# floswald/SMM.jl

Measured on AMD Instinct MI355X. Metric: chain-evals/sec (whole node), serialNormal 2p/2m, 4096 chains x 200 iters, higher is better.
Workload: dtype f64

## Files before the change

### smm.jl_amd/csrc/smm_chain_persist.hpp

```cpp
#pragma once
constexpr int PR_K = 8;
constexpr int PR_ZR = 20;
constexpr int PR_MAX_ITERS = 4000;
constexpr int PR_GATHER_DELAY = 8;
constexpr int PR_STW = 12;
constexpr unsigned long long PERSIST_TMO_FIRST = 40000000ull;

__host__ __device__ inline int persist_line(int np) { return PR_STW + ((3 + 2 * np + 1) & ~1); }

struct PrWin { uint32_t ctl, arrive, fin, progress, slot, rec; size_t total; };
__host__ __device__ inline PrWin pr_win_layout(const int Ng, const int RW, const int G, const int tiles_rank) {
    PrWin L;
    size_t o = 0;
    L.ctl = (uint32_t)o; o += 128;
    L.arrive = (uint32_t)o; o += (size_t)128 * P2P_MAXG;
    L.fin = (uint32_t)o; o += (size_t)128 * P2P_MAXG;
    L.progress = (uint32_t)o; o += (((size_t)G * tiles_rank * 4) + 127) & ~(size_t)127;
    L.slot = (uint32_t)o; o += ((size_t)PR_K * ((size_t)Ng + 4) * 8 + 127) & ~(size_t)127;
    L.rec = (uint32_t)o; o += ((size_t)PR_K * (size_t)Ng * RW * 16 + 127) & ~(size_t)127;
    L.total = o;
    return L;
}

struct PersistArgs {
// ... 9 lines not shown
    int ring_k, slow_tile, slow_ticks, walk_first, unit_sh, scout_after, scout_gl;
    uint32_t epoch;
    double sigma_adjust_by, thr;
    uint64_t seed;
    unsigned long long tmo;
    const double* mi_g;
    int u_lanes, n_udata;
    unsigned char* win[P2P_MAXG];
    uint32_t o_arrive;
    int G, rank, offset;
    int slow_read;
    uint32_t o_slot;
    int tables_local;
    const double* chol_L;
    int chol_per_chain;
};

__device__ inline uint32_t pr_tag16(const uint32_t epoch, const int rel) { return 0x8000u | ((epoch & 0x7fu) << 8) | ((uint32_t)rel & 0xffu); }
__device__ inline uint32_t pr_tag32(const uint32_t epoch, const int rel) { return 0x80000000u | ((epoch & 0x7ffffu) << 12) | ((uint32_t)rel & 0xfffu); }
__device__ inline uint32_t pr_progress_word(const uint32_t epoch, const int rel) { return (epoch << 12) | (uint32_t)rel; }

#define PR_SC "sc0 sc1"
__device__ inline unsigned long long pr_load8_sys(const void* p) {
    unsigned long long v;
    asm volatile("global_load_dwordx2 %0, %1, off " PR_SC "\n\ts_waitcnt vmcnt(0)" : "=v"(v) : "v"(p) : "memory");
    return v;
}
__device__ inline uint32_t pr_load4_sys(const void* p) { return __hip_atomic_load((const uint32_t*)p, __ATOMIC_RELAXED, __HIP_MEMORY_SCOPE_SYSTEM); }
__device__ inline uint4 pr_load16_sys(const void* p) {
    p2p_u32x4 q;
// ... 238 lines not shown
```

### smm.jl_amd/csrc/smm_chain_persist_loc.hpp

```cpp
#pragma once
constexpr int PL_LOCN = NORM_CT + CONE_GCAP + 2;
constexpr uint32_t PL_PBASE = ((16u * PL_LOCN + 127u) & ~127u);
constexpr int PL_HASH = 1024;
constexpr size_t PL_TSW_BASE = (size_t)8 * 8192;
constexpr int PL_TSW_TILES = 2048, PL_TSW = 8;
constexpr size_t PL_LATE_BASE = PL_TSW_BASE + (size_t)PL_TSW_TILES * (NORM_WG / 64) * PL_TSW;
constexpr int PL_LATE_N = 16384;
static_assert(PL_LATE_BASE + PL_LATE_N <= (size_t)8 * 60000, "the stamp buffer: the exchange kernels' words start at 8 * 60000");

__host__ __device__ inline size_t persist_loc_smem_bytes(const int np) {
    const size_t hw = (size_t)((H_PARAMS + 2 * np + 1) & ~1);
    const size_t dbl = (size_t)NORM_CT * np + (size_t)np * 8 * NORM_CT + (size_t)NORM_CT * persist_line(np) + 2 * 64 * (size_t)(1 + 2 * np) +
                       2 * NORM_CT * hw + (size_t)PR_ZR * 64 + 16 + 16 + 2 * 64 * 2 + (size_t)PL_LOCN * np + (size_t)PL_LOCN +
                       (size_t)(NORM_WG / 64) * PL_TSW;
    return (size_t)PL_PBASE + 2 * (size_t)CONE_LEVELS * 64 * 4 + 2 * (size_t)CONE_GCAP * 2 + 4 * 16 * 4 + 2 * (size_t)PL_HASH * 4 + dbl * 8;
}

template <int NP>
struct PersistLocLds {
    using L = NormLayout<NP>;
    static constexpr int CT = NORM_CT, RW = L::RW, HW = L::HW, LW = PR_STW + RW, RNGW = 1 + 2 * NP;
    uint32_t pbase, gbase, hbase, tbase;
    uint32_t* s_hdr;
    double *s_theta, *s_part, *s_st, *s_rng, *s_hrow, *s_xrow, *s_z0, *s_const, *s_gth, *s_thr;
    uint4* s_donor;
    unsigned long long *s_ts, *s_wts;
    unsigned* s_arrived; int* s_minprog; unsigned* s_abort; unsigned* s_xmask; int* s_glready; int* s_pub; int* s_hready;
    __device__ inline PersistLocLds(unsigned char* lds) {
        pbase = PL_PBASE;
        gbase = pbase + 2u * CONE_LEVELS * 64 * 4;
        hbase = gbase + 2u * CONE_GCAP * 2;
        tbase = hbase + 4u * 16 * 4;
        s_hdr = (uint32_t*)(lds + hbase);
        s_theta = (double*)(lds + tbase + 2u * PL_HASH * 4);
        s_part = s_theta + CT * NP;
        s_st = s_part + NP * 8 * CT;
        s_rng = s_st + CT * LW;
        s_hrow = s_rng + 2 * 64 * RNGW;
        s_xrow = s_hrow + CT * HW;
        s_z0 = s_xrow + CT * HW;
        s_const = s_z0 + PR_ZR * 64;
        s_ts = (unsigned long long*)(s_const + 16);
        s_arrived = (unsigned*)(s_ts + 8);
        s_minprog = (int*)(s_arrived + 1);
        s_abort = s_arrived + 2;
        s_xmask = s_arrived + 3;
        s_glready = (int*)(s_arrived + 4);
        s_pub = (int*)(s_arrived + 5);
        s_hready = (int*)(s_arrived + 6);
        s_donor = (uint4*)(s_const + 16 + 16);
        s_gth = s_const + 16 + 16 + 2 * 64 * 2;
        s_thr = s_gth + PL_LOCN * NP;
        s_wts = (unsigned long long*)(s_thr + PL_LOCN);
    }
};

__device__ inline uint32_t pl_hslot(const uint32_t chain) { return (chain * 2654435761u) >> 22; }
static_assert(PL_HASH == 1024, "pl_hslot: 10 bits");
__device__ inline void pl_hash_put(uint32_t* tab, const uint32_t chain, const uint32_t local) {
    uint32_t h = pl_hslot(chain);
    while (atomicCAS(&tab[h], 0u, ((chain + 1u) << 16) | local) != 0u) h = (h + 1u) & (PL_HASH - 1);
}
__device__ inline uint32_t pl_hash_get(const uint32_t* tab, const uint32_t chain) {
    uint32_t h = pl_hslot(chain);
    for (int probe = 0; probe < PL_HASH; ++probe) {
        const uint32_t v = tab[h];
        if ((v >> 16) == chain + 1u) return v & 0xffffu;
        if (v == 0u) break;
// ... 86 lines not shown
                for (int k = 0; k < NP; ++k) Y.s_gth[cl * NP + k] = A.rec_in[(size_t)c * RW + 3 + k];
                if constexpr (PCT) Y.s_thr[cl] = A.mi_g[c0g + (uint32_t)cl];
            }
        }
#pragma unroll
        for (int u = 0; u < PR_ZR; ++u) Y.s_z0[u * 64 + lane] = (lane + u * WG < A.ns) ? A.Z[lane + (size_t)u * WG] : 0.0;
    }
    if (tid >= 64 && tid < 64 + NP) {
        const int k = tid - 64;
        Y.s_const[k] = A.lb[k]; Y.s_const[NP + k] = A.ub[k]; Y.s_const[2 * NP + k] = A.mom[k]; Y.s_const[3 * NP + k] = A.w[k];
    }
    if (tid == 128) {
        Y.s_const[4 * NP] = A.failbox ? A.objp[0] : 1.0; Y.s_const[4 * NP + 1] = A.failbox ? A.objp[1] : 0.0;
        Y.s_const[4 * NP + 2] = (double)A.ns;
        *Y.s_arrived = 0u; *Y.s_minprog = 0; *Y.s_abort = 0u; *Y.s_xmask = 0u; *Y.s_glready = t0 - 2; *Y.s_pub = t0 - 2; *Y.s_hready = t0 - 2;
    }
    if (tid >= 192 && tid < 200) Y.s_ts[tid - 192] = 0ull;
    if (A.ts && tid >= 256 && tid < 256 + (NORM_WG / 64) * PL_TSW) Y.s_wts[tid - 256] = 0ull;
    if (wave == 3 && lane < CONE_HDRW) {
        if (A.walk_first) Y.s_hdr[((t0 - 1) & 3) * 16 + lane] = A.cone_hdr[((size_t)(t0 - 1 - A.plan_t0) * tiles + tile) * CONE_HDRW + lane];
        if (t0 < t1 && exch_on(t0)) Y.s_hdr[(t0 & 3) * 16 + lane] = A.cone_hdr[((size_t)(t0 - A.plan_t0) * tiles + tile) * CONE_HDRW + lane];
    }
    if constexpr (SH) {
        if (tile == 0 && wave == 2 && lane < A.G) {
            unsigned char* w = nullptr;
#pragma unroll
            for (int p = 0; p < P2P_MAXG; ++p) w = lane == p ? A.win[p] : w;
            __hip_atomic_store((uint32_t*)(w + A.o_arrive + 128 * (size_t)A.rank), epoch, __ATOMIC_RELAXED, __HIP_MEMORY_SCOPE_SYSTEM);
        }
        if (wave == 2) {
// ... 222 lines not shown
        };
        if (wave == 1 || (wave == 2 && PR_AHEAD > 1)) make_rng(t0, wave - 1);
        for (int t = t0; t <= t1; ++t) {
            const int rel = t - t0 + 1;
            PR_BARRIER();
            uint32_t nhdr = 0u;
            const bool want_hdr = wave == 3 && lane < CONE_HDRW && t + 1 < t1 && exch_on(t + 1);
            if (wave == 3) {
                if (t > t0) {
                    store_rows(Y.s_hrow, t - 1, 0xffffu);
                    store_rows(Y.s_xrow, t - 2, *Y.s_xmask);
                }
                if (want_hdr) nhdr = A.cone_hdr[((size_t)(t + 1 - A.plan_t0) * tiles + tile) * CONE_HDRW + lane];
            }
            if (t < t1 && exch_on(t)) request_lists(t);
            PR_BARRIER();
            unsigned long long tw0 = 0, tw1 = 0, tw2 = 0;
            if (A.ts) tw0 = wall_clock64();
            if (simw) {
                __builtin_amdgcn_s_setprio(1);
                if (nfull == PR_ZR - 1) persist_simulate<NP, true>(z, nfull, extra, Y.s_theta, Y.s_part, h, wih, A.ts != nullptr, tw1);
                else persist_simulate<NP, false>(z, nfull, extra, Y.s_theta, Y.s_part, h, wih, A.ts != nullptr, tw1);
                if (A.ts) tw2 = wall_clock64();
                __builtin_amdgcn_fence(__ATOMIC_RELEASE, "workgroup");
                const int lane3 = (int)__builtin_amdgcn_mbcnt_hi(~0u, __builtin_amdgcn_mbcnt_lo(~0u, 0u));
                if (lane3 == 0) __hip_atomic_fetch_add(Y.s_arrived, 1u, __ATOMIC_RELAXED, __HIP_MEMORY_SCOPE_WORKGROUP);
                __builtin_amdgcn_s_setprio(0);
            }
            const int lane = (int)__builtin_amdgcn_mbcnt_hi(~0u, __builtin_amdgcn_mbcnt_lo(~0u, 0u));
            const bool lists = t < t1 && exch_on(t);
            if (wave == 3 || wave >= 8) {
                if (wave == 3 && want_hdr) Y.s_hdr[((t + 1) & 3) * 16 + lane] = nhdr;
                asm volatile("s_waitcnt vmcnt(0)" ::: "memory");
                if (wave == 3 && lane == 0) __hip_atomic_store(Y.s_glready, t, __ATOMIC_RELEASE, __HIP_MEMORY_SCOPE_WORKGROUP);
                if (wave == 3 && lists) {
                    build_table(t, lane);
                    if (lane == 0) __hip_atomic_store(Y.s_hready, t, __ATOMIC_RELEASE, __HIP_MEMORY_SCOPE_WORKGROUP);
                }
                if (wave >= 8 && lists) {
                    if (!A.tables_local) while (__hip_atomic_load(Y.s_hready, __ATOMIC_ACQUIRE, __HIP_MEMORY_SCOPE_WORKGROUP) != t) __builtin_amdgcn_s_sleep(1);
                    fix_lists(t, t + 1, lane);
                }
            }
            if (wave == 2) {
                const int m = pr_min_progress(pr_progress, epoch, tiles_all, lane);
                if (lane == 0) {
                    __hip_atomic_store(Y.s_minprog, m, __ATOMIC_RELAXED, __HIP_MEMORY_SCOPE_WORKGROUP);
                    if (pr_load4_sys(pr_ctl) == epoch) *Y.s_abort = 1u;
                    if (lists && A.cone_ok[t - A.plan_t0] == 0u) pr_report(A.err, 3, t + 1, (int)c0g);
                }
                if constexpr (SH) {
                    if (*Y.s_abort && lane < A.G) {
                        unsigned char* w = nullptr;
#pragma unroll
                        for (int p = 0; p < P2P_MAXG; ++p) w = lane == p ? A.win[p] : w;
                        __hip_atomic_store((uint32_t*)(w + A.o_ctl), epoch, __ATOMIC_RELAXED, __HIP_MEMORY_SCOPE_SYSTEM);
// ... 22 lines not shown
                const double2* st2 = (const double2*)(Y.s_st + cl * LW);
                double2* g_cs = (double2*)(A.cs + (size_t)c * CSW);
                for (int i = r; i < 6; i += 4) g_cs[i] = i == 2 ? make_double2(st2[2].x, 0.0) : st2[i];
                for (int i = r; i < NPC; i += 4) ((double2*)(A.rec_out + (size_t)c * RW))[i] = st2[PR_STW / 2 + i];
                if (r == 0) {
                    const double v = Y.s_st[cl * LW + PR_STW];
                    A.vals_out[c] = v;
                    if (A.slot8_out) { A.slot8_out[c] = make_uint2(order_key32(v), (uint32_t)c); if (v != v) atomicOr(A.walk_flags, 1u); }
                }
            }
        }
        return;
    }

    const int nfull0 = A.ns / WG;
    for (int t = t0; t <= t1; ++t) {
        const int rel = t - t0 + 1;
        const bool exch = t == t0 ? A.walk_first != 0 : exch_on(t - 1);
        double z0[PR_ZR];
        uint32_t wmeta;
        PR_BARRIER();
        {
            const int lane = (int)__builtin_amdgcn_mbcnt_hi(~0u, __builtin_amdgcn_mbcnt_lo(~0u, 0u));
            const int cl = lane >> 2, r = lane & 3;
            const int c = tile * CT + cl;
            const bool valid = c < N;
            double* st = Y.s_st + cl * LW;
            unsigned long long ts1 = 0;
            if (A.ts && lane == 0) { ts1 = wall_clock64(); if (t != t0) Y.s_ts[0] += ts1 - Y.s_ts[7]; }
            wmeta = (uint32_t)cl;
            if (exch) {
                const uint32_t lbase = Y.pbase + (uint32_t)((t - 1) & 1) * (CONE_LEVELS * 64 * 4);
                uint32_t hw, pw0;
                lean_sub64_head(Y.hbase + (uint32_t)((t - 1) & 3) * 64u, lbase, lane, hw, pw0);
                const int nsub = (int)((uint32_t)__builtin_amdgcn_readfirstlane((int)hw) & 0xffffu);
                if constexpr (WIDE) {
                    lean_walk_sub64<0, true, WalkNoGuard, PCT>(lbase, nsub, lane, pw0, A.thr, WalkNoGuard(), (uint32_t)((unsigned char*)Y.s_thr - lds));
                } else {
                    const PersistLocWalkValues values{W, mine, A.o_rec, rel, rmask, A.Ng, Y.gbase + (uint32_t)((t - 1) & 1) * (CONE_GCAP * 2), c0g, RW, NP, t};
                    lean_walk_sub64<0, false, PersistLocWalkValues>(lbase, nsub, lane, pw0, 0.0, values);
                }
                if (valid) wmeta = WIDE ? ((const uint4*)lds)[cl].z : ((const uint2*)lds)[cl].y;
            }
            const uint32_t src = wmeta & 0xffffu;
            const bool donor = valid && src != (uint32_t)cl;
            unsigned long long ts2 = 0;
            if (A.ts && lane == 0) ts2 = wall_clock64();
            double mu01[NP], th[NP], th_old[NP];
            const double sigma = st[CS_SIGMA];
            const double* o = Y.s_rng + ((t & 1) * 64 + lane) * RNGW;
            bool found = !valid;
            {
                double x[NP];
                bool ok = valid;
#pragma unroll
                for (int k = 0; k < NP; ++k) {
                    const double lbk = Y.s_const[k], ubk = Y.s_const[NP + k];
                    th_old[k] = donor ? Y.s_gth[src * NP + k] : st[PR_STW + 3 + k];
                    th[k] = valid ? th_old[k] : 0.0;
                    mu01[k] = (th_old[k] - lbk) / (ubk - lbk);
                    const double step = sigma * o[1 + k];
                    x[k] = mu01[k] + step;
                    if (!(x[k] >= 0.0 && x[k] <= 1.0)) ok = false;
                }
                if (r >= A.smpl_iters || (A.user_n && r >= A.rb_tries)) ok = false;
                const unsigned long long m = __ballot(ok);
                const unsigned quad = (unsigned)(m >> (lane & ~3)) & 0xfu;
                if (quad) {
                    const int rwin = __builtin_ctz(quad);
#pragma unroll
                    for (int k = 0; k < NP; ++k) {
                        const double lbk = Y.s_const[k];
                        const double sc = x[k] * (Y.s_const[NP + k] - lbk);
                        const double thk = sc + lbk;
                        th[k] = quad_bcast_dyn(thk, lane, rwin);
                    }
                    found = true;
                }
            }
            if (__builtin_expect(__any(!found), 0)) {
                if (A.ts && lane == 0) Y.s_wts[7] -= wall_clock64();
                int j_next = NORM_NR;
                if (PR_AHEAD > 1 && (A.rb == nullptr || A.rb_tries >= 2 * NORM_NR)) {
                    double x[NP];
                    bool ok = !found;
#pragma unroll
                    for (int k = 0; k < NP; ++k) {
                        const double step = sigma * o[1 + NP + k];
                        x[k] = mu01[k] + step;
                        if (!(x[k] >= 0.0 && x[k] <= 1.0)) ok = false;
                    }
                    if (NORM_NR + r >= A.smpl_iters || (A.user_n && NORM_NR + r >= A.rb_tries)) ok = false;
                    const unsigned long long m = __ballot(ok);
                    const unsigned quad = (unsigned)(m >> (lane & ~3)) & 0xfu;
                    if (!found && quad) {
                        const int rwin = __builtin_ctz(quad);
#pragma unroll
                        for (int k = 0; k < NP; ++k) {
                            const double lbk = Y.s_const[k];
                            const double sc = x[k] * (Y.s_const[NP + k] - lbk);
                            const double thk = sc + lbk;
                            th[k] = quad_bcast_dyn(thk, lane, rwin);
                        }
                        found = true;
                    }
                    j_next = 2 * NORM_NR;
                }
                if (__any(!found)) {
                    const PrTries TR{A.rb, A.seed, A.rb_t0, A.N, A.RBW, A.rb_tries, A.user_n, A.smpl_iters, A.offset};
                    const PrTh<NP> lt = persist_late_tries<NP>(TR, o, t, c, valid, lane, found, sigma, mu01[0], mu01[NP - 1], Y.s_const, th[0], th[NP - 1], j_next);
#pragma unroll
                    for (int k = 0; k < NP; ++k) th[k] = lt.th[k];
                    found = lt.found;
                    if (!found && r == 0) pr_report(A.err, ERRK_NO_DRAW, t, (int)c0g + cl);
                }
                if (A.ts && lane == 0) {
// ... 57 lines not shown
            __builtin_amdgcn_s_setprio(0);
        }
        {
            const unsigned want = (unsigned)(8 * NP) * (unsigned)rel;
            while (__hip_atomic_load(Y.s_arrived, __ATOMIC_RELAXED, __HIP_MEMORY_SCOPE_WORKGROUP) < want) __builtin_amdgcn_s_sleep(1);
            __builtin_amdgcn_fence(__ATOMIC_ACQUIRE, "workgroup");
        }
        if (A.ts) tw3 = wall_clock64();
        const int lane = (int)__builtin_amdgcn_mbcnt_hi(~0u, __builtin_amdgcn_mbcnt_lo(~0u, 0u));
        const int cl = lane >> 2, r = lane & 3;
        const int c = tile * CT + cl;
        const bool valid = c < N;
        double* st = Y.s_st + cl * LW;
        unsigned long long ts5 = 0;
        if (A.ts && lane == 0) ts5 = wall_clock64();
        if (valid) {
            const int src = (int)st[CS_WASX];
            const bool donor = src != cl;
            double rc2[RW];
#pragma unroll
            for (int f = 0; f < RW; ++f) rc2[f] = st[PR_STW + f];
            if (donor) {
                asm volatile("s_waitcnt vmcnt(0)" ::: "memory");
                const uint32_t tag = pr_tag32(epoch, rel - 1);
                double rr[8];
#pragma unroll
                for (int f = 0; f < 8; ++f) rr[f] = 0.0;
                bool ok = true;
#pragma unroll
                for (int f = 0; f < RW; ++f) {
// ... 63 lines not shown
                if (r == 0) {
                    double* hx = Y.s_xrow + cl * HW;
                    swapped_head(hx, rc2, partner, b);
#pragma unroll
                    for (int k = 0; k < 2 * NP; ++k) hx[H_PARAMS + k] = rc2[3 + k];
                    if (HW > H_PARAMS + 2 * NP) hx[HW - 1] = 0.0;
                }
            } else { nn += 1; na += (int)st[CS_LACC]; }
            double nsig = sig;
            const bool upd = (t % A.sigma_update_steps) == 0;
            if (upd || t == t1) {
                const double rate = accept_rate(na, nn, acc);
                if (upd) nsig = sigma_next(sig, rate, A.sigma_adjust_by);
                if (r == 0) st[CS_RATE] = rate;
            }
            const double currv = acc ? value : old;
            const Best b = best_of(value, t, bp, bpid);
            const double bestv = b.best, bestid = b.best_id;
            if (r == 0) {
                if constexpr (WIDE) ((uint4*)lds)[cl] = make_uint4((uint32_t)__double2loint(v), (uint32_t)__double2hiint(v), (uint32_t)cl, 0u);
                else ((uint2*)lds)[cl] = make_uint2(order_key32(v), (uint32_t)cl);
#pragma unroll
                for (int k = 0; k < NP; ++k) Y.s_gth[cl * NP + k] = nr[3 + k];
                st[CS_SIGMA] = nsig; st[CS_NNOEX] = (double)nn; st[CS_NACC] = (double)na; st[CS_LACC] = accd;
                st[CS_BEST] = bestv; st[CS_BESTID] = bestid; st[CS_BESTP] = bp; st[CS_BESTPID] = bpid;
#pragma unroll
                for (int f = 0; f < RW; ++f) st[PR_STW + f] = nr[f];
                double* hv = Y.s_hrow + cl * HW;
                history_head(hv, value, prob, currv, bestv, bestid, 0.0, accd, (double)status);
#pragma unroll
// ... 3 lines not shown
        }
        {
            const unsigned long long xm = __ballot(valid && r == 0 && (int)st[CS_PARTNER] != 0);
            if (lane == 0) {
                unsigned m = 0u;
#pragma unroll
                for (int q = 0; q < CT; ++q) m |= (unsigned)((xm >> (4 * q)) & 1ull) << q;
                *Y.s_xmask = m;
            }
        }
        if (A.ts && lane == 0) { const unsigned long long ts7 = wall_clock64(); Y.s_ts[2] += ts7 - Y.s_ts[6]; Y.s_ts[7] = ts7; pl_wts_add(Y.s_wts, tw0, tw1, tw2, tw3); }
    }
    PR_BARRIER();
    {
        const int lane = (int)__builtin_amdgcn_mbcnt_hi(~0u, __builtin_amdgcn_mbcnt_lo(~0u, 0u));
        if (A.ts && lane < 7) A.ts[(size_t)tile * 8 + lane] = lane < 6 ? Y.s_ts[lane] : (unsigned long long)(t1 - t0 + 1);
        if (A.ts && lane == 0) pl_wts_out(A.ts, Y.s_wts, tile, 0);
    }
}
```

### smm.jl_amd/csrc/smm_run_host.hpp

```cpp
#pragma once

namespace {

void persist_repair(Ctx* c, int n_replay = -1);
void p2p_enqueue(Ctx* c, int n_iters);
unsigned long long p2p_agree_error(Ctx* c, unsigned long long e_local) {
    const KParams& P = c->P;
    const int G = P.p2p_G;
    const PrWin WL = pr_win_layout(P.Ng, P.RW, G, persist_tiles_rank(c->F, c->P.N));
    const uint32_t seq = c->pr_epoch;
    for (int r = 0; r < G; ++r)
        HIPCHK(hipMemcpy(P.p2p_win[r] + c->prw_off + WL.fin + 128 * (size_t)P.p2p_rank, &e_local, 8, hipMemcpyHostToDevice));
    for (int r = 0; r < G; ++r)
        HIPCHK(hipMemcpy(P.p2p_win[r] + c->prw_off + WL.fin + 128 * (size_t)P.p2p_rank + 8, &seq, 4, hipMemcpyHostToDevice));
    std::vector<unsigned char> buf((size_t)128 * G);
    const auto t0 = std::chrono::steady_clock::now();
    unsigned long long e = e_local;
    for (;;) {
        HIPCHK(hipMemcpy(buf.data(), c->p2p_mine + c->prw_off + WL.fin, buf.size(), hipMemcpyDeviceToHost));
        bool all = true;
        e = e_local;
        for (int r = 0; r < G; ++r) {
            uint32_t s_r; unsigned long long e_r;
            memcpy(&e_r, buf.data() + 128 * (size_t)r, 8); memcpy(&s_r, buf.data() + 128 * (size_t)r + 8, 4);
// ... 187 lines not shown
        for (int r = 0; r < G; ++r) A.win[r] = P.p2p_win[r] + c->prw_off;
        A.self = c->p2p_mine + c->prw_off;
    } else { A.win[0] = c->prw; A.self = c->prw; }
    A.o_ctl = WL.ctl; A.o_arrive = WL.arrive; A.o_progress = WL.progress; A.o_slot = WL.slot; A.o_rec = WL.rec;
    A.cs = P.cs; A.rec_in = c->rec[c->run.cur]; A.rec_out = c->rec[c->run.cur ^ 1]; A.vals_out = P.vals_out; A.slot8_out = P.slot8_out; A.walk_flags = P.walk_flags;
    A.hrec = P.hrec; A.err = P.err; A.ts = P.ts;
    A.Z = P.Z; A.lb = P.lb; A.ub = P.ub; A.mom = P.mom; A.w = P.w; A.objp = P.objp; A.dense_Bf = P.dense_Bf; A.dense_Af = P.dense_Af; A.dense_A2f = P.dense_A2f;
    A.rb = pregen ? P.rb : nullptr;
    A.mi_g = P.min_improve_g;
    A.N = P.N; A.Ng = P.Ng; A.np = P.np; A.nm = P.nm; A.ns = P.ns; A.zstride = P.zstride; A.RW = P.RW; A.HW = P.HW; A.RBW = P.RBW; A.dense_nOt = P.dense_nOt;
    A.batch_size = P.batch_size; A.failbox = (P.obj == SMM_OBJ_NORM_FAILBOX && P.objp) ? 1 : 0;
    A.G = G; A.rank = sh ? P.p2p_rank : 0; A.offset = P.offset;
    A.plan_t0 = P.plan_t0; A.exch_from = c->exchange_from; A.sigma_update_steps = P.sigma_update_steps; A.smpl_iters = P.smpl_iters; A.t0 = t0; A.t1 = t1;
    A.rb_t0 = P.rb_t0; A.rb_tries = P.rb_tries; A.user_n = P.user_n;
    A.ring_k = c->H.pr_ring_k; A.slow_tile = c->H.pr_slow_tile; A.slow_ticks = c->H.pr_slow_ticks; A.walk_first = c->run.unresolved ? 1 : 0;
    A.slow_read = c->H.pr_slow_read;
    A.tables_local = c->F.persist_sh_big ? 1 : 0; A.unit_sh = P.lean_unit == 16 ? 4 : (P.lean_unit == 8 ? 3 : 2); A.scout_after = P.scout_after; A.scout_gl = P.scout_gl;
    A.u_lanes = c->u_lanes; A.n_udata = c->n_objp;
    A.chol_L = P.chol_L; A.chol_per_chain = P.chol_per_chain;
    A.epoch = c->pr_epoch; A.sigma_adjust_by = P.sigma_adjust_by; A.thr = P.mi_value; A.seed = P.seed; A.tmo = tmo;
    return A;
}
int launch_chain_persist(Ctx* c, int n_left) {
    const int t0 = c->run.iter + 1;
    const bool pregen = (c->F.persist == PERSIST_GEN || c->F.persist == PERSIST_TILE) ? (c->P.user_ntab || c->P.user_utab) : !(c->F.norm_fast && !c->P.user_ntab && !c->P.user_utab);
    if ((c->F.persist == PERSIST_LOC || c->F.persist == PERSIST_TILE) && c->run.unresolved && !(t0 - 1 >= c->plan_t0 && t0 + 1 < c->plan_t0 + c->plan_w)) {
        c->plan_w = 0;
        ensure_windows(c, t0 - 1, pregen);
    } else if (!c->run.unresolved) ensure_windows(c, t0, pregen);
    if (pregen && !(t0 >= c->rng_t0 && t0 < c->rng_t0 + c->rng_w)) ensure_windows(c, t0);
    int t1 = std::min(c->run.iter + n_left, c->plan_t0 + c->plan_w - 1);
// ... 602 lines not shown
```

### smm.jl_amd/csrc/smm_walk_lean.hpp

```cpp
#pragma once
__host__ __device__ inline int lean_walk_Kp(int K) { return (K + 64 * LV_MAXLEV + 3) & ~3; }
typedef unsigned int u32x4_t __attribute__((ext_vector_type(4)));
typedef unsigned int u32x2_t __attribute__((ext_vector_type(2)));
enum { LEAN_KEYS = 0, LEAN_WIDE = 1, LEAN_TILE16 = 2 };
__host__ __device__ constexpr uint32_t lean_Ng4(int Ng) { return (uint32_t)((Ng + 3) & ~3); }
template <int LAY>
struct LeanLayout {
    static constexpr bool WIDE = LAY != LEAN_KEYS;
    static constexpr int SL = WIDE ? 4 : 3;
    static constexpr uint32_t SLOT = 1u << SL;
    static constexpr uint32_t PAD = LAY == LEAN_KEYS ? 4u : LAY == LEAN_WIDE ? 1u : 2u;
    static constexpr uint32_t DUMMIES = LAY == LEAN_WIDE ? 1u : 2u;
    __host__ __device__ static constexpr uint32_t pbase(uint32_t Ng4) { return SLOT * (Ng4 + PAD); }
    __host__ __device__ static constexpr uint32_t spare(uint32_t Ng4) {
        static_assert(LAY == LEAN_KEYS, "only the key layout has a spare slot: behind the dummies of the other two the pair words begin");
        return SLOT * (Ng4 + DUMMIES);
    }
    __host__ __device__ static constexpr size_t slot_bytes(int Ng) { return (size_t)pbase(lean_Ng4(Ng)); }
    __host__ __device__ static constexpr size_t bytes(int Ng, int K) { return slot_bytes(Ng) + (size_t)lean_walk_Kp(K) * 4; }
    __host__ __device__ static constexpr int unit4(uint32_t Ng4) { return SLOT * (Ng4 + DUMMIES) <= 65536u ? (int)SLOT : (int)SLOT / 2; }
    __host__ __device__ static constexpr int unit(int Ng) { return unit4(lean_Ng4(Ng)); }
    __host__ __device__ static constexpr uint32_t dummy_word(uint32_t unit, uint32_t Ng4) {
        return DUMMIES == 1u ? (unit * Ng4) * 0x10001u : (unit * Ng4) | ((unit * (Ng4 + 1u)) << 16);
    }
// ... 202 lines not shown
    using L = LeanLayout<LAY>;
    if (BYTES || unit == (int)L::SLOT) lean_walk_levels<NT, 0, L::WIDE, GUARD>(vsrc, vstride, L::pbase(Ng4), ov, nlev, tid, ltail, thr, guard);
    else lean_walk_levels<NT, 1, L::WIDE, GUARD>(vsrc, vstride, L::pbase(Ng4), ov, nlev, tid, ltail, thr, guard);
}
template <int LAY>
__device__ inline unsigned long long lean_result(const unsigned char* lds, const uint32_t Ng4, const int unit, const uint32_t g) {
    using L = LeanLayout<LAY>;
    const uint32_t meta = *(const uint32_t*)(lds + L::SLOT * g + (L::WIDE ? 8u : 4u));
    const uint32_t partner = unit == (int)L::SLOT ? lean_partner<0, L::SL>(lds, L::pbase(Ng4), meta, g) : lean_partner<1, L::SL>(lds, L::pbase(Ng4), meta, g);
    return (unsigned long long)(meta & 0xffffu) | ((unsigned long long)partner << 32);
}

__device__ inline void lean_sub64_head(const uint32_t hoff, const uint32_t pbase, const int lane, uint32_t& hdr, uint32_t& pw) {
    asm volatile("ds_read_b32 %0, %2\n\tds_read_b32 %1, %3\n\ts_waitcnt lgkmcnt(0)" : "=&v"(hdr), "=&v"(pw) : "v"(hoff), "v"(pbase + 4u * (uint32_t)lane) : "memory");
}
#define LEAN_SUB64_OFF(o) " offset:" #o "\n\t"
template <int US, bool WIDE, class GUARD, bool PCT, int OFF>
__device__ __forceinline__ void lean_sub64_level(const uint32_t ptr, const uint32_t stamp, uint32_t& pw, const double thr, const GUARD& guard, const uint32_t thr_base) {
    static_assert(OFF == 256 || OFF == 512 || OFF == 768 || OFF == 1024, "the word of the next sub-level within a trip of four");
    uint32_t ai, aj;
    lean_decode<US>(pw, ai, aj);
    uint32_t pwn;
    if constexpr (WIDE) {
        u32x4_t si, sj;
        double thr_l = thr;
#define LEAN_SUB64_WIDE(o) \
        if constexpr (PCT)  \
            asm volatile("ds_read_b128 %0, %4\n\tds_read_b128 %1, %5\n\tds_read_b32 %2, %6" LEAN_SUB64_OFF(o) "ds_read_b64 %3, %7\n\ts_waitcnt lgkmcnt(0)" \
                         : "=&v"(si), "=&v"(sj), "=&v"(pwn), "=&v"(thr_l) : "v"(ai), "v"(aj), "v"(ptr), "v"(thr_base + (ai >> 1)) : "memory"); \
        else \
// ... 16 lines not shown
        else if constexpr (OFF == 768) { LEAN_SUB64_KEY(768); } else { LEAN_SUB64_KEY(1024); }
#undef LEAN_SUB64_KEY
        bool swap = si.x > sj.x;
        const bool tie = si.x == sj.x;
        if (__builtin_expect(__ballot(tie) != 0ull, 0)) {
            if (tie) swap = walk_value(guard, nullptr, 1, si.y & 0xffffu) - walk_value(guard, nullptr, 1, sj.y & 0xffffu) > 0.0;
        }
        if (swap) {
            const u32x2_t ni = {sj.x, (sj.y & 0xffffu) | stamp}, nj = {si.x, (si.y & 0xffffu) | stamp};
            asm volatile("ds_write_b64 %0, %2\n\tds_write_b64 %1, %3" :: "v"(ai), "v"(aj), "v"(ni), "v"(nj) : "memory");
        }
    }
    pw = pwn;
}
#undef LEAN_SUB64_OFF
template <int US, bool WIDE = false, class GUARD = WalkNoGuard, bool PCT = false>
__device__ inline void lean_walk_sub64(const uint32_t pbase, const int nsub, const int lane, uint32_t pw, const double thr = 0.0, const GUARD& guard = GUARD(),
                                       const uint32_t thr_base = 0u) {
    static_assert(!std::is_same<GUARD, WalkNoGuard>::value || WIDE, "a key tie reads the exact values through the guard: there is no plain array here");
    constexpr uint32_t SUBST = 64u << 16;
    uint32_t ptr = pbase + 4u * (uint32_t)lane;
    uint32_t stamp = ((uint32_t)lane + 1u) << 16;
    int left = nsub;
#pragma clang loop unroll(disable)
    for (; left >= 4; left -= 4) {
        lean_sub64_level<US, WIDE, GUARD, PCT, 256>(ptr, stamp, pw, thr, guard, thr_base);
        lean_sub64_level<US, WIDE, GUARD, PCT, 512>(ptr, stamp + SUBST, pw, thr, guard, thr_base);
        lean_sub64_level<US, WIDE, GUARD, PCT, 768>(ptr, stamp + 2u * SUBST, pw, thr, guard, thr_base);
        lean_sub64_level<US, WIDE, GUARD, PCT, 1024>(ptr, stamp + 3u * SUBST, pw, thr, guard, thr_base);
        ptr += 1024u; stamp += 4u * SUBST;
    }
    if (left & 2) {
        lean_sub64_level<US, WIDE, GUARD, PCT, 256>(ptr, stamp, pw, thr, guard, thr_base);
        lean_sub64_level<US, WIDE, GUARD, PCT, 512>(ptr, stamp + SUBST, pw, thr, guard, thr_base);
        ptr += 512u; stamp += 2u * SUBST;
    }
    if (left & 1) lean_sub64_level<US, WIDE, GUARD, PCT, 256>(ptr, stamp, pw, thr, guard, thr_base);
    asm volatile("s_waitcnt lgkmcnt(0)" ::: "memory");
}
```

### smm.jl_amd/csrc/smmhip.hip

```cpp
#include <hip/hip_runtime.h>
#include <hip/hip_ext.h>
#include <hip/hiprtc.h>
#include <dlfcn.h>
#include <chrono>
#include <mutex>
#include <thread>
#include <stdint.h>
#include <stdio.h>
#include <string.h>
#include <stdlib.h>
#include <math.h>
#include <algorithm>
#include <string>
#include <vector>
#include <type_traits>

#include "../../include/smmhip.h"
#include "smm_rng.hpp"

namespace {

using namespace smm;

#include "smm_params.hpp"
// ... 44 lines not shown
    bool key_walk_off = false;
    bool inline_walk_off = false;
    bool norm_fast_off = false;
    int norm_narrow = -1;
    int tpw = 0;
    bool dense_keys_off = false;
    bool no_cone = false;
    bool persist_off = false, persist_loc_off = false, persist_tile_off = false;
    bool cone_big_off = false;
    bool plan_ahead_off = false;
    int plan_cap = 1 << 30;
    int lvl_wg = 1024;
    int scout_after = SMM_SCOUT_AFTER, scout_gl = 16;
    int a2a_cap = 0;
    int pr_ring_k = PR_K, pr_slow_tile = -1, pr_slow_ticks = 0;
    int pr_slow_read = 0;
    bool rows_win_check = false;
    size_t stats_scratch = 0;
    int stats_mode_bins = STATS_MODE_BINS;
    long long group_wide_min = STATS_LDS_N + 1;
    int hist_lds_bins = 1 << 30;
    size_t pop_scratch = 0;
    size_t opt_scratch = 0;
    bool opt_materialise = false;
};
Hooks read_hooks() {
    Hooks H;
    auto is = [](const char* v, char ch) { return v && v[0] == ch; };
    if (const char* v = SMM_HOOK("SMMHIP_FILL")) H.fill = atoi(v);
    H.any_exchange = is(SMM_HOOK("SMMHIP_ANY_EXCHANGE"), '1');
// ... 9 lines not shown
    H.no_cone = is(SMM_HOOK("SMMHIP_NO_CONE"), '1');
    H.persist_off = is(SMM_HOOK("SMMHIP_PERSIST"), '0');
    H.persist_loc_off = is(SMM_HOOK("SMMHIP_PERSIST_LOC"), '0');
    H.persist_tile_off = is(SMM_HOOK("SMMHIP_PERSIST_TILE"), '0');
    H.cone_big_off = is(SMM_HOOK("SMMHIP_CONE_BIG"), '0');
    H.plan_ahead_off = is(SMM_HOOK("SMMHIP_PLAN_AHEAD"), '0');
    if (const char* v = SMM_HOOK("SMMHIP_PLAN_CAP")) H.plan_cap = atoi(v);
    if (const char* v = SMM_HOOK("SMMHIP_LVL_WG")) H.lvl_wg = atoi(v);
    if (const char* v = SMM_HOOK("SMMHIP_SCOUT_AFTER")) H.scout_after = atoi(v);
    if (const char* v = SMM_HOOK("SMMHIP_SCOUT_GL")) H.scout_gl = atoi(v) == 8 ? 8 : 16;
    if (const char* v = SMM_HOOK("SMMHIP_A2A_CAP")) H.a2a_cap = std::max(1, atoi(v));
    if (const char* v = SMM_HOOK("SMMHIP_PR_RING")) { const int k = atoi(v); if (k == 2 || k == 4) H.pr_ring_k = k; }
    if (const char* v = SMM_HOOK("SMMHIP_PR_SLOW_TILE")) H.pr_slow_tile = atoi(v);
    if (const char* v = SMM_HOOK("SMMHIP_PR_SLOW_US")) H.pr_slow_ticks = 100 * atoi(v);
    H.pr_slow_read = is(SMM_HOOK("SMMHIP_PR_SLOW_READ"), '1');
    H.rows_win_check = SMM_HOOK("SMMHIP_ROWS_WIN_CHECK") != nullptr;
    if (const char* v = SMM_HOOK("SMMHIP_STATS_SCRATCH")) H.stats_scratch = (size_t)strtoull(v, nullptr, 10);
    if (const char* v = SMM_HOOK("SMMHIP_STATS_MODE_BINS")) H.stats_mode_bins = std::min(STATS_MODE_BINS, std::max(1, atoi(v)));
    if (const char* v = SMM_HOOK("SMMHIP_GROUP_WIDE_MIN")) H.group_wide_min = std::min((long long)STATS_LDS_N + 1, std::max(1ll, atoll(v)));
    if (const char* v = SMM_HOOK("SMMHIP_HIST_LDS_BINS")) H.hist_lds_bins = std::max(1, atoi(v));
    if (const char* v = SMM_HOOK("SMMHIP_POP_SCRATCH")) H.pop_scratch = (size_t)strtoull(v, nullptr, 10);
    if (const char* v = SMM_HOOK("SMMHIP_OPT_SCRATCH")) H.opt_scratch = (size_t)strtoull(v, nullptr, 10);
    H.opt_materialise = is(SMM_HOOK("SMMHIP_OPT_MATERIALISE"), '1');
    return H;
}
enum ExchKernel { XK_LEAN, XK_LVL, XK_LVL_SOA, XK_TICKETS, XK_ROWS, XK_KEY, XK_LVL_BIG, XK_ANY };
enum PlanKind { PLAN_NONE, PLAN_LDS, PLAN_BIG };
enum PersistKind { PERSIST_NONE, PERSIST_GEN, PERSIST_LOC, PERSIST_TILE };
struct Forms {
    PlanKind plan = PLAN_NONE;
// ... 553 lines not shown
```

Measured before the change: 361.1 million.

## Hoist per-step walk setup and donor normalisation ahead of the persist barrier

Moves the walk header read, pointer setup, bounds and normalised own-parameter computation in the persistent local chain kernel before the per-step barrier, so that work overlaps with waiting. Helper waves precompute normalised donor parameters into a new LDS array, and the list-fix waves publish ready counters. The walker consumes these only when the counters match, otherwise it rereads or recomputes. Sigma and own theta are carried in registers across steps instead of being reread from LDS. This adds LDS space, counter synchronisation and fallback paths, which risk subtle ordering bugs.

```diff
diff --git a/smm.jl_amd/csrc/smm_chain_persist.hpp b/smm.jl_amd/csrc/smm_chain_persist.hpp
--- a/smm.jl_amd/csrc/smm_chain_persist.hpp
+++ b/smm.jl_amd/csrc/smm_chain_persist.hpp
@@ -47,6 +47,7 @@
     int tables_local;
     const double* chol_L;
     int chol_per_chain;
+    int ba_look;
 };
 
 __device__ inline uint32_t pr_tag16(const uint32_t epoch, const int rel) { return 0x8000u | ((epoch & 0x7fu) << 8) | ((uint32_t)rel & 0xffu); }
diff --git a/smm.jl_amd/csrc/smm_chain_persist_loc.hpp b/smm.jl_amd/csrc/smm_chain_persist_loc.hpp
--- a/smm.jl_amd/csrc/smm_chain_persist_loc.hpp
+++ b/smm.jl_amd/csrc/smm_chain_persist_loc.hpp
@@ -2,6 +2,8 @@
 constexpr int PL_LOCN = NORM_CT + CONE_GCAP + 2;
 constexpr uint32_t PL_PBASE = ((16u * PL_LOCN + 127u) & ~127u);
 constexpr int PL_HASH = 1024;
+constexpr uint32_t PL_MW = 4;
+constexpr uint32_t PL_LW = 8;
 constexpr size_t PL_TSW_BASE = (size_t)8 * 8192;
 constexpr int PL_TSW_TILES = 2048, PL_TSW = 8;
 constexpr size_t PL_LATE_BASE = PL_TSW_BASE + (size_t)PL_TSW_TILES * (NORM_WG / 64) * PL_TSW;
@@ -11,7 +13,7 @@
 __host__ __device__ inline size_t persist_loc_smem_bytes(const int np) {
     const size_t hw = (size_t)((H_PARAMS + 2 * np + 1) & ~1);
     const size_t dbl = (size_t)NORM_CT * np + (size_t)np * 8 * NORM_CT + (size_t)NORM_CT * persist_line(np) + 2 * 64 * (size_t)(1 + 2 * np) +
-                       2 * NORM_CT * hw + (size_t)PR_ZR * 64 + 16 + 16 + 2 * 64 * 2 + (size_t)PL_LOCN * np + (size_t)PL_LOCN +
+                       2 * NORM_CT * hw + (size_t)PR_ZR * 64 + 16 + 16 + 2 * 64 * 2 + 2 * (size_t)PL_LOCN * np + (size_t)PL_LOCN +
                        (size_t)(NORM_WG / 64) * PL_TSW;
     return (size_t)PL_PBASE + 2 * (size_t)CONE_LEVELS * 64 * 4 + 2 * (size_t)CONE_GCAP * 2 + 4 * 16 * 4 + 2 * (size_t)PL_HASH * 4 + dbl * 8;
 }
@@ -22,10 +24,11 @@
     static constexpr int CT = NORM_CT, RW = L::RW, HW = L::HW, LW = PR_STW + RW, RNGW = 1 + 2 * NP;
     uint32_t pbase, gbase, hbase, tbase;
     uint32_t* s_hdr;
-    double *s_theta, *s_part, *s_st, *s_rng, *s_hrow, *s_xrow, *s_z0, *s_const, *s_gth, *s_thr;
+    double *s_theta, *s_part, *s_st, *s_rng, *s_hrow, *s_xrow, *s_z0, *s_const, *s_gth, *s_thr, *s_gmu;
     uint4* s_donor;
     unsigned long long *s_ts, *s_wts;
-    unsigned* s_arrived; int* s_minprog; unsigned* s_abort; unsigned* s_xmask; int* s_glready; int* s_pub; int* s_hready;
+    unsigned* s_arrived; int* s_minprog; unsigned* s_abort; unsigned* s_xmask; int* s_glready; int* s_pub; int* s_hready; unsigned* s_lready; unsigned* s_mready;
+    unsigned long long* s_tsh;
     __device__ inline PersistLocLds(unsigned char* lds) {
         pbase = PL_PBASE;
         gbase = pbase + 2u * CONE_LEVELS * 64 * 4;
@@ -48,10 +51,14 @@
         s_glready = (int*)(s_arrived + 4);
         s_pub = (int*)(s_arrived + 5);
         s_hready = (int*)(s_arrived + 6);
+        s_lready = s_arrived + 7;
+        s_mready = s_arrived + 10;
+        s_tsh = (unsigned long long*)(s_arrived + 8);
         s_donor = (uint4*)(s_const + 16 + 16);
         s_gth = s_const + 16 + 16 + 2 * 64 * 2;
         s_thr = s_gth + PL_LOCN * NP;
-        s_wts = (unsigned long long*)(s_thr + PL_LOCN);
+        s_gmu = s_thr + PL_LOCN;
+        s_wts = (unsigned long long*)(s_gmu + PL_LOCN * NP);
     }
 };
 
@@ -168,6 +175,7 @@
         Y.s_const[4 * NP] = A.failbox ? A.objp[0] : 1.0; Y.s_const[4 * NP + 1] = A.failbox ? A.objp[1] : 0.0;
         Y.s_const[4 * NP + 2] = (double)A.ns;
         *Y.s_arrived = 0u; *Y.s_minprog = 0; *Y.s_abort = 0u; *Y.s_xmask = 0u; *Y.s_glready = t0 - 2; *Y.s_pub = t0 - 2; *Y.s_hready = t0 - 2;
+        *Y.s_lready = 0u; *Y.s_mready = 0u; *Y.s_tsh = 0ull;
     }
     if (tid >= 192 && tid < 200) Y.s_ts[tid - 192] = 0ull;
     if (A.ts && tid >= 256 && tid < 256 + (NORM_WG / 64) * PL_TSW) Y.s_wts[tid - 256] = 0ull;
@@ -420,6 +428,18 @@
                 if (want_hdr) nhdr = A.cone_hdr[((size_t)(t + 1 - A.plan_t0) * tiles + tile) * CONE_HDRW + lane];
             }
             if (t < t1 && exch_on(t)) request_lists(t);
+            if (wave >= 4 && wave < 8 && (t == t0 ? A.walk_first != 0 : exch_on(t - 1))) {
+                const int ngat = (int)(Y.s_hdr[((t - 1) & 3) * 16] >> 16);
+                for (int e = tid - 256; e < ngat; e += 256) {
+#pragma unroll
+                    for (int k = 0; k < NP; ++k) {
+                        const double lbk = Y.s_const[k], ubk = Y.s_const[NP + k];
+                        Y.s_gmu[(CT + e) * NP + k] = (Y.s_gth[(CT + e) * NP + k] - lbk) / (ubk - lbk);
+                    }
+                }
+                __builtin_amdgcn_fence(__ATOMIC_RELEASE, "workgroup");
+                if (lane == 0) __hip_atomic_fetch_add(Y.s_mready, 1u, __ATOMIC_RELAXED, __HIP_MEMORY_SCOPE_WORKGROUP);
+            }
             PR_BARRIER();
             unsigned long long tw0 = 0, tw1 = 0, tw2 = 0;
             if (A.ts) tw0 = wall_clock64();
@@ -446,6 +466,8 @@
                 if (wave >= 8 && lists) {
                     if (!A.tables_local) while (__hip_atomic_load(Y.s_hready, __ATOMIC_ACQUIRE, __HIP_MEMORY_SCOPE_WORKGROUP) != t) __builtin_amdgcn_s_sleep(1);
                     fix_lists(t, t + 1, lane);
+                    __builtin_amdgcn_fence(__ATOMIC_RELEASE, "workgroup");
+                    if (lane == 0) __hip_atomic_fetch_add(Y.s_lready, 1u, __ATOMIC_RELAXED, __HIP_MEMORY_SCOPE_WORKGROUP);
                 }
             }
             if (wave == 2) {
@@ -498,65 +520,125 @@
     }
 
     const int nfull0 = A.ns / WG;
+    double c_sigma, c_own[NP];
+    {
+        const double* st = Y.s_st + (lane >> 2) * LW;
+        c_sigma = st[CS_SIGMA];
+#pragma unroll
+        for (int k = 0; k < NP; ++k) c_own[k] = st[PR_STW + 3 + k];
+    }
+    uint32_t lwant = 0u, mwant = 0u;
     for (int t = t0; t <= t1; ++t) {
         const int rel = t - t0 + 1;
         const bool exch = t == t0 ? A.walk_first != 0 : exch_on(t - 1);
         double z0[PR_ZR];
         uint32_t wmeta;
-        PR_BARRIER();
+        if (t == t0) PR_BARRIER();
+        uint32_t pw0 = 0u, wptr = 0u, wstamp = 0u;
+        int nsub = 0;
+        bool pw_ok = true;
+        double lbv[NP], span[NP], mu_own[NP];
+        bool try_ok;
+        {
+            const int lane = (int)__builtin_amdgcn_mbcnt_hi(~0u, __builtin_amdgcn_mbcnt_lo(~0u, 0u));
+            if (exch) {
+                const uint32_t lbase = Y.pbase + (uint32_t)((t - 1) & 1) * (CONE_LEVELS * 64 * 4);
+                uint32_t cnt, hw;
+                lean_sub64_head_look((uint32_t)((unsigned char*)Y.s_lready - lds), Y.hbase + (uint32_t)((t - 1) & 3) * 64u, lbase, lane, cnt, hw, pw0);
+                nsub = (int)((uint32_t)__builtin_amdgcn_readfirstlane((int)hw) & 0xffffu);
+                if (t != t0) {
+                    lwant += PL_LW;
+                    pw_ok = (uint32_t)__builtin_amdgcn_readfirstlane((int)cnt) == lwant;
+#ifdef SMM_TEST_HOOKS
+                    if (A.ba_look == 1 || (A.ba_look == 2 && (t & 1))) pw_ok = false;
+#endif
+                }
+                lean_sub64_start(lbase, lane, wptr, wstamp);
+            }
+            const int r = lane & 3;
+#pragma unroll
+            for (int k = 0; k < NP; ++k) {
+                lbv[k] = Y.s_const[k];
+                span[k] = Y.s_const[NP + k] - lbv[k];
+                mu_own[k] = (c_own[k] - lbv[k]) / span[k];
+            }
+            try_ok = !(r >= A.smpl_iters || (A.user_n && r >= A.rb_tries));
+            if (exch && r == 0) {
+#pragma unroll
+                for (int k = 0; k < NP; ++k) Y.s_gmu[(lane >> 2) * NP + k] = mu_own[k];
+            }
+            asm volatile("" : "+v"(pw0), "+v"(wptr), "+v"(wstamp), "+s"(nsub));
+#pragma unroll
+            for (int k = 0; k < NP; ++k) asm volatile("" : "+v"(lbv[k]), "+v"(span[k]), "+v"(mu_own[k]));
+            if (A.ts && lane == 0 && t != t0) { const unsigned long long tsh = wall_clock64(); *Y.s_tsh += tsh - Y.s_ts[7]; Y.s_ts[7] = tsh; }
+        }
+        if (t != t0) PR_BARRIER();
         {
             const int lane = (int)__builtin_amdgcn_mbcnt_hi(~0u, __builtin_amdgcn_mbcnt_lo(~0u, 0u));
             const int cl = lane >> 2, r = lane & 3;
             const int c = tile * CT + cl;
             const bool valid = c < N;
-            double* st = Y.s_st + cl * LW;
             unsigned long long ts1 = 0;
+            bool mu_ok = false;
             if (A.ts && lane == 0) { ts1 = wall_clock64(); if (t != t0) Y.s_ts[0] += ts1 - Y.s_ts[7]; }
             wmeta = (uint32_t)cl;
             if (exch) {
-                const uint32_t lbase = Y.pbase + (uint32_t)((t - 1) & 1) * (CONE_LEVELS * 64 * 4);
-                uint32_t hw, pw0;
-                lean_sub64_head(Y.hbase + (uint32_t)((t - 1) & 3) * 64u, lbase, lane, hw, pw0);
-                const int nsub = (int)((uint32_t)__builtin_amdgcn_readfirstlane((int)hw) & 0xffffu);
+                if (__builtin_expect(!pw_ok, 0)) pw0 = lean_sub64_word(Y.pbase + (uint32_t)((t - 1) & 1) * (CONE_LEVELS * 64 * 4), lane);
                 if constexpr (WIDE) {
-                    lean_walk_sub64<0, true, WalkNoGuard, PCT>(lbase, nsub, lane, pw0, A.thr, WalkNoGuard(), (uint32_t)((unsigned char*)Y.s_thr - lds));
+                    lean_walk_sub64_from<0, true, WalkNoGuard, PCT>(wptr, wstamp, nsub, pw0, A.thr, WalkNoGuard(), (uint32_t)((unsigned char*)Y.s_thr - lds));
                 } else {
                     const PersistLocWalkValues values{W, mine, A.o_rec, rel, rmask, A.Ng, Y.gbase + (uint32_t)((t - 1) & 1) * (CONE_GCAP * 2), c0g, RW, NP, t};
-                    lean_walk_sub64<0, false, PersistLocWalkValues>(lbase, nsub, lane, pw0, 0.0, values);
+                    lean_walk_sub64_from<0, false, PersistLocWalkValues>(wptr, wstamp, nsub, pw0, 0.0, values);
                 }
                 if (valid) wmeta = WIDE ? ((const uint4*)lds)[cl].z : ((const uint2*)lds)[cl].y;
+                mwant += PL_MW;
+                mu_ok = (uint32_t)__builtin_amdgcn_readfirstlane((int)__hip_atomic_load(Y.s_mready, __ATOMIC_ACQUIRE, __HIP_MEMORY_SCOPE_WORKGROUP)) == mwant;
+#ifdef SMM_TEST_HOOKS
+                if (A.ba_look == 1 || (A.ba_look == 2 && (t & 1))) mu_ok = false;
+#endif
             }
             const uint32_t src = wmeta & 0xffffu;
             const bool donor = valid && src != (uint32_t)cl;
             unsigned long long ts2 = 0;
             if (A.ts && lane == 0) ts2 = wall_clock64();
             double mu01[NP], th[NP], th_old[NP];
-            const double sigma = st[CS_SIGMA];
+            const double sigma = c_sigma;
             const double* o = Y.s_rng + ((t & 1) * 64 + lane) * RNGW;
             bool found = !valid;
             {
                 double x[NP];
                 bool ok = valid;
 #pragma unroll
+                for (int k = 0; k < NP; ++k) { th_old[k] = c_own[k]; mu01[k] = mu_own[k]; }
+                if (donor) {
+#pragma unroll
+                    for (int k = 0; k < NP; ++k) {
+                        th_old[k] = Y.s_gth[src * NP + k];
+                        mu01[k] = Y.s_gmu[src * NP + k];
+                    }
+                }
+                if (__builtin_expect(exch && !mu_ok, 0)) {
+                    if (donor) {
+#pragma unroll
+                        for (int k = 0; k < NP; ++k) mu01[k] = (th_old[k] - lbv[k]) / span[k];
+                    }
+                }
+#pragma unroll
                 for (int k = 0; k < NP; ++k) {
-                    const double lbk = Y.s_const[k], ubk = Y.s_const[NP + k];
-                    th_old[k] = donor ? Y.s_gth[src * NP + k] : st[PR_STW + 3 + k];
                     th[k] = valid ? th_old[k] : 0.0;
-                    mu01[k] = (th_old[k] - lbk) / (ubk - lbk);
                     const double step = sigma * o[1 + k];
                     x[k] = mu01[k] + step;
                     if (!(x[k] >= 0.0 && x[k] <= 1.0)) ok = false;
                 }
-                if (r >= A.smpl_iters || (A.user_n && r >= A.rb_tries)) ok = false;
+                if (!try_ok) ok = false;
                 const unsigned long long m = __ballot(ok);
                 const unsigned quad = (unsigned)(m >> (lane & ~3)) & 0xfu;
                 if (quad) {
                     const int rwin = __builtin_ctz(quad);
 #pragma unroll
                     for (int k = 0; k < NP; ++k) {
-                        const double lbk = Y.s_const[k];
-                        const double sc = x[k] * (Y.s_const[NP + k] - lbk);
-                        const double thk = sc + lbk;
+                        const double sc = x[k] * span[k];
+                        const double thk = sc + lbv[k];
                         th[k] = quad_bcast_dyn(thk, lane, rwin);
                     }
                     found = true;
@@ -581,9 +663,8 @@
                         const int rwin = __builtin_ctz(quad);
 #pragma unroll
                         for (int k = 0; k < NP; ++k) {
-                            const double lbk = Y.s_const[k];
-                            const double sc = x[k] * (Y.s_const[NP + k] - lbk);
-                            const double thk = sc + lbk;
+                            const double sc = x[k] * span[k];
+                            const double thk = sc + lbv[k];
                             th[k] = quad_bcast_dyn(thk, lane, rwin);
                         }
                         found = true;
@@ -671,6 +752,9 @@
         double* st = Y.s_st + cl * LW;
         unsigned long long ts5 = 0;
         if (A.ts && lane == 0) ts5 = wall_clock64();
+        c_sigma = 0.0;
+#pragma unroll
+        for (int k = 0; k < NP; ++k) c_own[k] = 0.0;
         if (valid) {
             const int src = (int)st[CS_WASX];
             const bool donor = src != cl;
@@ -764,6 +848,9 @@
                 if (upd) nsig = sigma_next(sig, rate, A.sigma_adjust_by);
                 if (r == 0) st[CS_RATE] = rate;
             }
+            c_sigma = nsig;
+#pragma unroll
+            for (int k = 0; k < NP; ++k) c_own[k] = nr[3 + k];
             const double currv = acc ? value : old;
             const Best b = best_of(value, t, bp, bpid);
             const double bestv = b.best, bestid = b.best_id;
@@ -797,7 +884,7 @@
     PR_BARRIER();
     {
         const int lane = (int)__builtin_amdgcn_mbcnt_hi(~0u, __builtin_amdgcn_mbcnt_lo(~0u, 0u));
-        if (A.ts && lane < 7) A.ts[(size_t)tile * 8 + lane] = lane < 6 ? Y.s_ts[lane] : (unsigned long long)(t1 - t0 + 1);
+        if (A.ts && lane < 8) A.ts[(size_t)tile * 8 + lane] = lane < 6 ? Y.s_ts[lane] : lane == 6 ? (unsigned long long)(t1 - t0 + 1) : *Y.s_tsh;
         if (A.ts && lane == 0) pl_wts_out(A.ts, Y.s_wts, tile, 0);
     }
 }
diff --git a/smm.jl_amd/csrc/smm_run_host.hpp b/smm.jl_amd/csrc/smm_run_host.hpp
--- a/smm.jl_amd/csrc/smm_run_host.hpp
+++ b/smm.jl_amd/csrc/smm_run_host.hpp
@@ -225,7 +225,7 @@
     A.plan_t0 = P.plan_t0; A.exch_from = c->exchange_from; A.sigma_update_steps = P.sigma_update_steps; A.smpl_iters = P.smpl_iters; A.t0 = t0; A.t1 = t1;
     A.rb_t0 = P.rb_t0; A.rb_tries = P.rb_tries; A.user_n = P.user_n;
     A.ring_k = c->H.pr_ring_k; A.slow_tile = c->H.pr_slow_tile; A.slow_ticks = c->H.pr_slow_ticks; A.walk_first = c->run.unresolved ? 1 : 0;
-    A.slow_read = c->H.pr_slow_read;
+    A.slow_read = c->H.pr_slow_read; A.ba_look = c->H.pr_ba_look;
     A.tables_local = c->F.persist_sh_big ? 1 : 0; A.unit_sh = P.lean_unit == 16 ? 4 : (P.lean_unit == 8 ? 3 : 2); A.scout_after = P.scout_after; A.scout_gl = P.scout_gl;
     A.u_lanes = c->u_lanes; A.n_udata = c->n_objp;
     A.chol_L = P.chol_L; A.chol_per_chain = P.chol_per_chain;
diff --git a/smm.jl_amd/csrc/smm_walk_lean.hpp b/smm.jl_amd/csrc/smm_walk_lean.hpp
--- a/smm.jl_amd/csrc/smm_walk_lean.hpp
+++ b/smm.jl_amd/csrc/smm_walk_lean.hpp
@@ -240,6 +240,15 @@
 __device__ inline void lean_sub64_head(const uint32_t hoff, const uint32_t pbase, const int lane, uint32_t& hdr, uint32_t& pw) {
     asm volatile("ds_read_b32 %0, %2\n\tds_read_b32 %1, %3\n\ts_waitcnt lgkmcnt(0)" : "=&v"(hdr), "=&v"(pw) : "v"(hoff), "v"(pbase + 4u * (uint32_t)lane) : "memory");
 }
+__device__ inline void lean_sub64_head_look(const uint32_t coff, const uint32_t hoff, const uint32_t pbase, const int lane, uint32_t& cnt, uint32_t& hdr, uint32_t& pw) {
+    asm volatile("ds_read_b32 %0, %3\n\tds_read_b32 %1, %4\n\tds_read_b32 %2, %5\n\ts_waitcnt lgkmcnt(0)"
+                 : "=&v"(cnt), "=&v"(hdr), "=&v"(pw) : "v"(coff), "v"(hoff), "v"(pbase + 4u * (uint32_t)lane) : "memory");
+}
+__device__ inline uint32_t lean_sub64_word(const uint32_t pbase, const int lane) {
+    uint32_t pw;
+    asm volatile("ds_read_b32 %0, %1\n\ts_waitcnt lgkmcnt(0)" : "=v"(pw) : "v"(pbase + 4u * (uint32_t)lane) : "memory");
+    return pw;
+}
 #define LEAN_SUB64_OFF(o) " offset:" #o "\n\t"
 template <int US, bool WIDE, class GUARD, bool PCT, int OFF>
 __device__ __forceinline__ void lean_sub64_level(const uint32_t ptr, const uint32_t stamp, uint32_t& pw, const double thr, const GUARD& guard, const uint32_t thr_base) {
@@ -286,13 +295,15 @@
     pw = pwn;
 }
 #undef LEAN_SUB64_OFF
+__device__ inline void lean_sub64_start(const uint32_t pbase, const int lane, uint32_t& ptr, uint32_t& stamp) {
+    ptr = pbase + 4u * (uint32_t)lane;
+    stamp = ((uint32_t)lane + 1u) << 16;
+}
 template <int US, bool WIDE = false, class GUARD = WalkNoGuard, bool PCT = false>
-__device__ inline void lean_walk_sub64(const uint32_t pbase, const int nsub, const int lane, uint32_t pw, const double thr = 0.0, const GUARD& guard = GUARD(),
-                                       const uint32_t thr_base = 0u) {
+__device__ inline void lean_walk_sub64_from(uint32_t ptr, uint32_t stamp, const int nsub, uint32_t pw, const double thr = 0.0, const GUARD& guard = GUARD(),
+                                            const uint32_t thr_base = 0u) {
     static_assert(!std::is_same<GUARD, WalkNoGuard>::value || WIDE, "a key tie reads the exact values through the guard: there is no plain array here");
     constexpr uint32_t SUBST = 64u << 16;
-    uint32_t ptr = pbase + 4u * (uint32_t)lane;
-    uint32_t stamp = ((uint32_t)lane + 1u) << 16;
     int left = nsub;
 #pragma clang loop unroll(disable)
     for (; left >= 4; left -= 4) {
@@ -310,3 +321,10 @@
     if (left & 1) lean_sub64_level<US, WIDE, GUARD, PCT, 256>(ptr, stamp, pw, thr, guard, thr_base);
     asm volatile("s_waitcnt lgkmcnt(0)" ::: "memory");
 }
+template <int US, bool WIDE = false, class GUARD = WalkNoGuard, bool PCT = false>
+__device__ inline void lean_walk_sub64(const uint32_t pbase, const int nsub, const int lane, const uint32_t pw, const double thr = 0.0, const GUARD& guard = GUARD(),
+                                       const uint32_t thr_base = 0u) {
+    uint32_t ptr, stamp;
+    lean_sub64_start(pbase, lane, ptr, stamp);
+    lean_walk_sub64_from<US, WIDE, GUARD, PCT>(ptr, stamp, nsub, pw, thr, guard, thr_base);
+}
diff --git a/smm.jl_amd/csrc/smmhip.hip b/smm.jl_amd/csrc/smmhip.hip
--- a/smm.jl_amd/csrc/smmhip.hip
+++ b/smm.jl_amd/csrc/smmhip.hip
@@ -82,6 +82,7 @@
     int scout_after = SMM_SCOUT_AFTER, scout_gl = 16;
     int a2a_cap = 0;
     int pr_ring_k = PR_K, pr_slow_tile = -1, pr_slow_ticks = 0;
+    int pr_ba_look = 0;
     int pr_slow_read = 0;
     bool rows_win_check = false;
     size_t stats_scratch = 0;
@@ -121,6 +122,7 @@
     if (const char* v = SMM_HOOK("SMMHIP_PR_SLOW_TILE")) H.pr_slow_tile = atoi(v);
     if (const char* v = SMM_HOOK("SMMHIP_PR_SLOW_US")) H.pr_slow_ticks = 100 * atoi(v);
     H.pr_slow_read = is(SMM_HOOK("SMMHIP_PR_SLOW_READ"), '1');
+    if (const char* v = SMM_HOOK("SMMHIP_PR_BA_LOOK")) { const int m = atoi(v); if (m == 1 || m == 2) H.pr_ba_look = m; }
     H.rows_win_check = SMM_HOOK("SMMHIP_ROWS_WIN_CHECK") != nullptr;
     if (const char* v = SMM_HOOK("SMMHIP_STATS_SCRATCH")) H.stats_scratch = (size_t)strtoull(v, nullptr, 10);
     if (const char* v = SMM_HOOK("SMMHIP_STATS_MODE_BINS")) H.stats_mode_bins = std::min(STATS_MODE_BINS, std::max(1, atoi(v)));
```

Measured after the change: 361.9 million, median of 5. About the same (+0.2%).
